# Triton-AI/Triton-Racer-Sim

Hardware: AMD Instinct MI355X
Metric: env-steps/s (whole node) at N envs x 120x160 RGB (higher is better)
Workload: dtype f32 state / f64 nearest-point / u8 image; 1 GPU; 1024 envs/GPU x 1 GPU, bicycle physics + L1 nearest point + 120x160 RGB pinhole rasteriser = BASELINE configs[2], generated_track 1185 pts, synthetic controls seed 0x5EED, auto-reset; envs_total=1024, envs_per_gpu=1024, img_h=120, img_w=160, depth=False, steps_per_launch=1, step_mode=resident worker (posted steps), prewarm_steps=8400, launcher=self

## Files before the change

triton-racer-sim_amd/csrc/trsim_plan.hpp:

```cpp
#pragma once
#include <cstddef>
#include <string>
#include <vector>

#include "trsim_tables.hpp"

#ifndef TRS_RASTER_WAVES
#define TRS_RASTER_WAVES 8
#endif

namespace trsim {

constexpr int kRasterThreads = 64 * TRS_RASTER_WAVES;
constexpr int kPhysBlock = 256;
constexpr int kCamDepth = 4;
constexpr int kSlotWords = 20;
constexpr int kLensPalBytes = 513 * 16;
constexpr int kDynTabWords = 512 + 768 + 4 + 256;

using Variant = unsigned;
constexpr Variant kVDepth = 1, kVDyn = 2, kVHills = 4, kVLens = 8, kVLight = 16, kVariants = 32;
constexpr Variant variant_bits(bool depth, bool dyn, bool hills, bool lens, bool light)
{
    return (depth ? kVDepth : 0u) | (dyn ? kVDyn : 0u) | (hills ? kVHills : 0u) | (lens ? kVLens : 0u) | (light ? kVLight : 0u);
}
constexpr bool variant_built(Variant v) { return !((v & kVDyn) && (v & kVHills)) && !((v & kVLens) && (v & (kVDyn | kVHills | kVLight))); }

inline Variant variant_clash(Variant state, Variant add)
{
    if (variant_built(state | add)) return 0;
    for (const Variant b : {kVHills, kVDyn, kVLens, kVLight})
        if ((state & b) && !variant_built(add | b)) return b;
    return 0;
}
inline const char* variant_refusal(Variant add, Variant set)
{
    struct Text { Variant add, set; const char* text; };
    static const Text kTexts[] = {
        {kVHills, kVLens, "this track has elevation and a lens camera is set: the lens camera is built for flat tracks only (trs_set_camera(NULL) first); the handle keeps its track"},
        {kVHills, kVDyn, "this track has elevation: the dynamic-brightness frame filter that was set has been removed (a frame's palette is evaluated per env inside the kernels there; "
                         "the static filter works, or use trs_preprocess on the rendered frames)"},
        {kVDyn, kVHills, "the loaded track has elevation: a frame's palette is evaluated per env inside the kernels there, and the dynamic-brightness filter behind the "
                         "rasteriser is not built for that; the static filter works, or use trs_preprocess on the rendered frames"},
        {kVDyn, kVLens, "a lens camera is set: the dynamic-brightness filter behind the rasteriser is not built for the lens camera (trs_set_camera(NULL) first); "
                        "the static filter works, or use trs_preprocess on the rendered frames"},
        {kVLens, kVHills, "the loaded track has elevation: the lens camera is built for flat tracks only (the ground plane of a hilly track tilts per env and frame)"},
        {kVLens, kVDyn, "the dynamic-brightness frame filter is set: it is not built for the lens camera (trs_set_frame_filter without dynamic brightness, or NULL, first)"},
        {kVLens, kVLight, "scene lighting is set: it is not built for the lens camera (trs_set_lighting(NULL) first)"},
        {kVLight, kVLens, "a lens camera is set: scene lighting is not built for the lens camera (trs_set_camera(NULL) first)"},
    };
    for (const Text& t : kTexts)
        if (t.add == add && t.set == set) return t.text;
    return "";
}

constexpr int kHillRowBytes = 28;
constexpr int kHillBatchMax = 4;
TRS_HD inline int hill_table_bytes(int H) { return (kHillRowBytes * H + 15) & ~15; }
TRS_HD inline int hill_batch(int H) { const int b = kRasterThreads / (H > 0 ? H : 1); return b < 1 ? 1 : (b > kHillBatchMax ? kHillBatchMax : b); }
TRS_HD inline int hill_lds_bytes(int H) { return hill_batch(H) * hill_table_bytes(H) + 48; }

constexpr int kDynBatch = 4;
TRS_HD inline int light_copies(int gpr) { return (gpr + 63 + 63) / 64; }
TRS_HD inline int light_pal_bytes(int H, int gpr) { return light_copies(gpr) * H * 16; }
TRS_HD inline int light_lds_extra(int H, int W, int slots, bool hilly, bool dyn)
{
    return slots * 32 + (hilly ? 0 : (dyn ? kDynBatch * H * 16 : light_pal_bytes(H, W / 4)));
}
TRS_HD inline int dyn_lds_bytes(int H) { return kDynBatch * H * 16 + 128 + ((kDynTabWords * 4 + 15) & ~15) + H * 16; }

TRS_HD inline int imax(int a, int b) { return (a > b) ? a : b; }
struct StepLds { int cam, prog, pitch, hill, light, dyn, total; };
TRS_HD inline int tabs_lds_bytes(int H, Variant v) { return (v & kVHills) ? hill_lds_bytes(H) : ((v & kVLens) ? kLensPalBytes : 0); }
TRS_HD inline StepLds step_lds_behind(int prog, int epw, int H, Variant v, int n_phys)
{
    const int rows = imax(n_phys, 1) + 1;
    StepLds L;
    L.prog = prog;
    L.cam = prog - rows * epw * 16;
    L.pitch = L.prog + epw * 4 + 16;
    L.hill = (L.pitch + rows * epw * 4 + 15) & ~15;
    L.light = (L.hill + tabs_lds_bytes(H, v) + 15) & ~15;
    return L;
}
TRS_HD inline StepLds step_lds_layout(int lds_step, int epw, int H, int W, Variant v, int n_phys)
{
    StepLds L = step_lds_behind(lds_step + (imax(n_phys, 1) + 1) * epw * 16, epw, H, v, n_phys);
    int end = L.pitch;
    if (v & (kVHills | kVLens | kVLight)) end = L.hill + tabs_lds_bytes(H, v);
    if (v & kVLight) end = L.light + light_lds_extra(H, W, epw, (v & kVHills) != 0, (v & kVDyn) != 0);
    L.dyn = (end + 15) & ~15;
    L.total = (v & kVDyn) ? L.dyn + dyn_lds_bytes(H) : end;
    return L;
}

TRS_HD inline size_t wlds_slot_off(int epw) { return (64 + (size_t)epw * 8 + 15) & ~(size_t)15; }
TRS_HD inline size_t wlds_bytes(int epw)
{
    return wlds_slot_off(epw) + (size_t)kCamDepth * epw * kSlotWords * 4 + (size_t)epw * 64;
}

struct WorkerLds { int ctl, dyn, hill, light, total; };
TRS_HD inline int worker_lds_light(int hill, int H, Variant v) { return (hill + tabs_lds_bytes(H, v) + 15) & ~15; }
TRS_HD inline WorkerLds worker_lds_layout(int lds_step, int epw, int H, int W, Variant v)
{
    WorkerLds L;
    L.ctl = (lds_step + 15) & ~15;
    int end = (int)(L.ctl + wlds_bytes(epw) + 16);
    L.dyn = (end + 15) & ~15;
    if (v & kVDyn) end = L.dyn + dyn_lds_bytes(H);
    L.hill = (end + 15) & ~15;
    if (v & (kVHills | kVLens)) end = L.hill + tabs_lds_bytes(H, v);
    L.light = worker_lds_light(L.hill, H, v);
    L.total = (v & kVLight) ? L.light + light_lds_extra(H, W, kCamDepth * epw, (v & kVHills) != 0, (v & kVDyn) != 0) : end;
    return L;
}

inline int steps_that_fit(int lds_step, int epw, int H, int W, Variant v)
{
    int n = 0;
    while (n < 16 && step_lds_layout(lds_step, epw, H, W, v, n + 1).total <= 160 * 1024) ++n;
    return n;
}
inline bool resident_fits(int lds_step, int epw, int H, int W, Variant v) { return worker_lds_layout(lds_step, epw, H, W, v).total <= 160 * 1024; }
enum class LdsFit { ok, no_launch, no_worker };
inline LdsFit lds_fit(int lds_step, int epw, int H, int W, Variant v, bool resident)
{
    if (steps_that_fit(lds_step, epw, H, W, v) < 1) return LdsFit::no_launch;
    return resident && !resident_fits(lds_step, epw, H, W, v) ? LdsFit::no_worker : LdsFit::ok;
}

constexpr bool variant_keeps_uniform(Variant v) { return !(v & (kVDyn | kVLens | kVLight)); }
struct UniformRows {
    bool ok[2] = {false, false};
    void invalidate() { ok[0] = ok[1] = false; }
    unsigned skip_mask(Variant v) const { return variant_keeps_uniform(v) ? (ok[0] ? 1u : 0u) | (ok[1] ? 2u : 0u) : 0u; }
    void rendered(Variant v, unsigned long long first, unsigned long long n)
    {
        for (unsigned long long k = 0; k < n && k < 2; ++k) ok[(first + k) & 1ull] = variant_keeps_uniform(v);
    }
};

TRS_HD inline bool worker_skips_uniform(unsigned mask, unsigned long long start, unsigned long long s) { return ((mask >> (s & 1ull)) & 1u) != 0 || s - start >= 2; }
TRS_HD inline int worker_step_stores(int nstep, int nuni, bool skips) { return skips ? nstep - nuni : nstep; }
TRS_HD inline int worker_wait_count(unsigned mask, unsigned long long start, unsigned long long owed, unsigned long long s, int nstep, int nuni, int uni_now)
{
    int n = uni_now;
    for (unsigned long long q = owed + 1; q < s; ++q) n += worker_step_stores(nstep, nuni, worker_skips_uniform(mask, start, q));
    return n;
}
TRS_HD inline int worker_lag(int nstep, int nuni, bool skipping) { return (2 * worker_step_stores(nstep, nuni, skipping) + (skipping ? 0 : nuni) <= 63) ? 3 : 2; }

struct TrackLayout {
    struct Phys { int off_py, off_pz, off_tan, tan_in_lds, off_gstart, off_gpts, blob_bytes, off_scratch, pts_bytes, lds_p; } p;
    struct Raster { int map_pitch_b, off_rowtab, off_pal, off_depth, off_sky, blob_bytes, lds_r; } r;
    int lds_off_phys, lds_step;
};
int track_layout(const TrackTables& T, int H, bool render, int envs_per_wg, TrackLayout& L, std::string& err);
void pack_track_images(const TrackTables& T, int H, const TrackLayout& L, std::vector<unsigned char>& phys, std::vector<unsigned char>& raster);

}
```

triton-racer-sim_amd/csrc/trsim_resident.hip:

```cpp
#include <hip/hip_runtime.h>

#include <algorithm>
#include <array>
#include <atomic>
#include <chrono>
#include <cstdint>
#include <cstdlib>
#include <cstddef>
#include <cstring>
#include <mutex>
#include <string>
#include <utility>

#include "../../include/trsim.h"
#include "../../include/trsim_spec.h"
#include "trsim_device.hpp"
#include "trsim_env.hpp"
#include "trsim_internal.hpp"

#define TRS_EXPORT extern "C" __attribute__((visibility("default")))

namespace trsim {

constexpr int kSlots = 8;
// ... 220 lines not shown
        seen = ok ? (want | 0x100u) : expected;
    }
    seen = (unsigned)__builtin_amdgcn_readfirstlane((int)seen);
    won = (seen & 0x100u) != 0u;
    return seen & 0xffu;
}

__device__ __forceinline__ void leave_not_coresident(const WParams& wp, const WLds& l, int lane, bool won)
{
    if (won) {
        if (lane == 0) sys_store64(&wp.mb->consumed, wp.start);
        drain_vmem();
        if (lane == 0) sys_store64(&wp.mb->exited, kExitNotCoresident);
    }
    dispatcher_publish_exit(wp, l, wp.start, lane);
}

__device__ __forceinline__ int dispatcher_checkin(const WParams& wp, const WLds& l, int lane)
{
    const u64 t0 = (u64)wall_clock64();
    bool cancel = sys_load64(&wp.mb->close) == kCloseCancel, won = false;
    for (unsigned spins = 0; !cancel; ++spins) {
        if (decision_load(wp) == kNoGo) { leave_not_coresident(wp, l, lane, false); return 0; }
        if (__hip_atomic_load(&wp.dc->checkin[0], __ATOMIC_RELAXED, __HIP_MEMORY_SCOPE_AGENT) >= (unsigned)wp.n_blocks) {
            if (decision_close(wp, kGo, lane, won) != kGo) { leave_not_coresident(wp, l, lane, false); return 0; }
            if (lane == 0) sys_store64(&wp.mb->started, 1ull);
            return 1;
        }
        if (agent_load64(&wp.dc->word) & kAbortBit) {
            if (lane == 0) __hip_atomic_fetch_or(l.word, kAbortBit, __ATOMIC_RELAXED, __HIP_MEMORY_SCOPE_WORKGROUP);
            return 0;
        }
        if ((u64)wall_clock64() - t0 > wp.checkin_ticks) break;
        if ((spins & 63u) == 63u) cancel = sys_load64(&wp.mb->close) == kCloseCancel;
        __builtin_amdgcn_s_sleep(4);
    }
    const unsigned d = decision_close(wp, kNoGo, lane, won);
    if (d == kGo) { if (lane == 0) sys_store64(&wp.mb->started, 1ull); return 1; }
    leave_not_coresident(wp, l, lane, won);
    return 0;
}

__device__ __forceinline__ int leader_wait_decision(const WParams& wp, const WLds& l, int lane)
{
    const u64 t0 = (u64)wall_clock64();
    for (;;) {
        unsigned d = decision_load(wp);
        if (d == 0u && (u64)wall_clock64() - t0 > 2ull * wp.checkin_ticks) {
            bool won = false;
            d = decision_close(wp, kNoGo, lane, won);
            if (d == kNoGo) { leave_not_coresident(wp, l, lane, won); return 0; }
        }
        if (d == kGo) return 1;
        if (d == kNoGo) { leave_not_coresident(wp, l, lane, false); return 0; }
        if (agent_load64(&wp.dc->word) & kAbortBit) {
            if (lane == 0) __hip_atomic_fetch_or(l.word, kAbortBit, __ATOMIC_RELAXED, __HIP_MEMORY_SCOPE_WORKGROUP);
            return 0;
        }
        __builtin_amdgcn_s_sleep(8);
    }
}

__device__ __forceinline__ void dispatcher_run(const WParams& wp, const WLds& l, int lane)
{
    if (!dispatcher_checkin(wp, l, lane)) return;
    Leader L{wp.start, (u64)wall_clock64(), (u64)wall_clock64()};
    for (;;) {
        if ((lds_load64(l.word) | agent_load64(&wp.dc->word)) & kAbortBit) {
            if (lane == 0) __hip_atomic_fetch_or(l.word, kAbortBit, __ATOMIC_RELAXED, __HIP_MEMORY_SCOPE_WORKGROUP);
            return;
        }
        const u64 now = (u64)wall_clock64();
        bool close_req = false;
        const int fresh = dispatcher_take(wp, l, L, lane, close_req);
        const bool busy = (u64)lds_load64(l.fwd) < L.known;
        if (fresh || busy) L.t_last = now;
        const bool leave = (!fresh && (close_req || now - L.t_last > wp.idle_ticks)) || now - L.t_start > wp.life_ticks;
        if (!leave) { if (!fresh) __builtin_amdgcn_s_sleep(4); continue; }
        if (lane == 0) sys_store64(&wp.mb->exited, kExitNormal);
        drain_vmem();
        (void)dispatcher_take(wp, l, L, lane, close_req);
        if (lane == 0) sys_store64(&wp.mb->consumed, L.known);
        dispatcher_publish_exit(wp, l, L.known, lane);
        return;
    }
}

__device__ __forceinline__ void raster_arrive(const WLds& l, u64 s, int lane)
{
    if (lane == 0) __hip_atomic_fetch_add(&l.arrive[s & (kSlots - 1)], 1, __ATOMIC_RELAXED, __HIP_MEMORY_SCOPE_WORKGROUP);
}

__device__ __forceinline__ void forward_arrivals(const WParams& wp, const WLds& l, u64& fwd, int lane, int want = kRasterThreads / 64)
{
    const int slot = (int)(fwd & (kSlots - 1));
    if (lds_load32(&l.arrive[slot]) != want) return;
    if (lane == 0) {
        lds_store32(&l.arrive[slot], 0);
        const int shard = (int)(blockIdx.x & 7u), nshards = min(8, wp.n_blocks);
        const unsigned members = (unsigned)((wp.n_blocks - shard + 7) / 8);
        const unsigned uses = (unsigned)((fwd - wp.start) / (u64)kSlots) + 1u;
        unsigned* a = &wp.dc->arrive[slot][shard][0];
        if (__hip_atomic_fetch_add(a, 1u, __ATOMIC_RELAXED, __HIP_MEMORY_SCOPE_AGENT) == members * uses - 1u) {
            unsigned* t = &wp.dc->top[slot][0];
            if (__hip_atomic_fetch_add(t, 1u, __ATOMIC_RELAXED, __HIP_MEMORY_SCOPE_AGENT) == (unsigned)nshards * uses - 1u)
                sys_store64(&wp.mb->done[slot], fwd + 1);
        }
    }
    fwd += 1;
    if (lane == 0) lds_store64(l.fwd, fwd);
}

struct Duties { bool leader, forwarder; u64 fwd; int want = kRasterThreads / 64; };

__device__ __forceinline__ int wait_posted(const WParams& wp, const WLds& l, Duties& D, u64 s, int lane)
{
    u64 t0 = 0;
    for (unsigned spins = 0;; ++spins) {
        if (D.forwarder) forward_arrivals(wp, l, D.fwd, lane, D.want);
        const u64 w = lds_load64(l.word);
        if (w & kAbortBit) return 0;
        if ((w & kCountMask) > s) return 1;
        if (w & kExitBit) return 0;
        if (D.leader) {
            const u64 g = agent_load64(&wp.dc->word);
            if (g != w) { if (lane == 0) lds_store64(l.word, g); drain_lds(); continue; }
        }
        __builtin_amdgcn_s_sleep(4);
        if ((spins & 255u) == 255u) {
            const u64 now = (u64)wall_clock64();
            if (t0 == 0) t0 = now;
            else if (now - t0 > wp.safety_ticks) { worker_abort(wp, l, 1u); return 0; }
        }
    }
}

__device__ __forceinline__ int wait_lds_ge(const WParams& wp, const WLds& l, Duties* D, const int* ctr, int want, unsigned code, int lane)
{
    u64 t0 = 0;
    for (unsigned spins = 0;; ++spins) {
        if (lds_load32(ctr) >= want) return 1;
        if (D && D->forwarder) forward_arrivals(wp, l, D->fwd, lane, D->want);
        __builtin_amdgcn_s_sleep(1);
        if ((spins & 1023u) == 1023u) {
            if (lds_load64(l.word) & kAbortBit) return 0;
            const u64 now = (u64)wall_clock64();
            if (t0 == 0) t0 = now;
            else if (now - t0 > wp.safety_ticks) { worker_abort(wp, l, code); return 0; }
        }
    }
}

template <bool DEPTH, bool DYN, bool HILLS = false, bool LENS = false, bool LIGHT = false>
__global__ __launch_bounds__(kBlock) void trs_worker_kernel(const WParams wp)
{
    const int tid = threadIdx.x, lane = tid & 63, wave = tid >> 6;
    const bool raster_team = tid < kRasterThreads;
    const RParams& p = wp.ra;
    const PParams& P = wp.ph;
    const int epw = p.envs_per_wg;
    const WLds l = wlds_of(smem + wp.lds_off_ctl, epw);
    const int e_begin = blockIdx.x * epw;
    const int n_loc = min(e_begin + epw, p.n_envs) - e_begin;
    const int pw = wave - kRasterThreads / 64;
    if ((unsigned)(uintptr_t)smem != 0u) {
        if (tid == 0) {
            atomicAdd(&p.stats[2], 1ull);
            sys_store64(p.fault, 1ull);
            sys_store64(&wp.mb->error, (9ull << 32) | (u64)blockIdx.x);
            __hip_atomic_fetch_or(&wp.dc->word, kAbortBit, __ATOMIC_RELAXED, __HIP_MEMORY_SCOPE_AGENT);
            if (blockIdx.x == 0) { sys_store64(&wp.mb->consumed, wp.start); sys_store64(&wp.mb->exited, 1ull); }
        }
        return;
    }
    if (raster_team) stage_lds_dma(p.blob, p.blob_bytes, 0u, wave, kRasterThreads / 64, lane);
    else stage_lds_dma(P.blob, P.blob_bytes, (unsigned)wp.lds_off_phys, pw, kPhysWaves, lane);
    if (LENS && raster_team) lens_stage_palette(p, (unsigned)wp.lds_off_hill, wave, lane);
    if (tid == 0) { lds_store64(l.word, wp.start); lds_store64(l.fwd, wp.start); }
    if (tid < kSlots) l.arrive[tid] = 0;
    for (int j = tid; j < 2 * epw; j += kBlock) l.pprog[j] = 0;
    int* const hbar = reinterpret_cast<int*>(smem + wp.lds_off_hill + hill_batch(p.H) * hill_table_bytes(p.H));
    if (HILLS && tid == 0) *hbar = 0;
    const int lds_off_light = worker_lds_light(wp.lds_off_hill, p.H, variant_bits(DEPTH, DYN, HILLS, LENS, LIGHT));
    float* const lring = reinterpret_cast<float*>(smem + lds_off_light);
    const unsigned lds_off_lpal = (unsigned)lds_off_light + (unsigned)(kCamDepth * epw * 32);
    const float* const light_g = LIGHT ? reinterpret_cast<const trsim::HillBlock*>(p.blob + trsim::hill_block_offset(p.blob_bytes))->light : nullptr;
    const int lfilt = LIGHT ? reinterpret_cast<const trsim::HillBlock*>(p.blob + trsim::hill_block_offset(p.blob_bytes))->filt : 0;
    if constexpr (DYN) {
        if (tid < 32) reinterpret_cast<int*>(smem + wp.fp.lds_off + kDynBatch * p.H * 16)[tid] = 0;
        dyn_stage_tables(smem, wp.fp, p.H, tid, kBlock, reinterpret_cast<const uint32_t*>(p.blob + p.off_pal));
    }
    if (!raster_team)
        for (int j = pw; j < n_loc; j += kPhysWaves) {
            EnvRegs st;
            env_load(P, e_begin + j, st);
            const float lr = coherent_load(&P.last_return[e_begin + j]);
            if (lane == 0) {
                float* q = l.lst + (size_t)j * 16;
                q[0] = st.x; q[1] = st.y; q[2] = st.z; q[3] = st.yaw; q[4] = st.v; q[5] = st.sf; q[6] = st.epr;
                q[7] = __int_as_float(st.seg); q[8] = __int_as_float(st.epl); q[9] = __int_as_float(st.done); q[10] = __int_as_float(st.pend);
                q[11] = lr;
            }
        }
    asm volatile("s_waitcnt vmcnt(0) lgkmcnt(0)" ::: "memory");
    __syncthreads();
    if (tid == 0) worker_checkin(wp);

    if (!raster_team) {
        const int first = blockIdx.x == 0 ? 1 : 0, nphys = kPhysWaves - first;
        if (pw < first) { dispatcher_run(wp, l, lane); return; }
        Duties D{blockIdx.x != 0 && pw == 0, pw == kPhysWaves - 1, wp.start};
        if (D.leader && !leader_wait_decision(wp, l, lane)) return;
        const unsigned char* const lphys = smem + wp.lds_off_phys;
        u64 s = wp.start;
        for (;; ++s) {
            const int r = (int)(s - wp.start);
            if (!wait_posted(wp, l, D, s, lane)) break;
            const u64* en = reinterpret_cast<const u64*>(&wp.dc->ring[s & (kSlots - 1)]);
            const u64 ev = lane < 6 ? agent_load64(en + lane) : 0ull;
            const float* const c_st = reinterpret_cast<const float*>(lane_u64(ev, 1));
            const float* const c_th = reinterpret_cast<const float*>(lane_u64(ev, 2));
            const float* const c_br = reinterpret_cast<const float*>(lane_u64(ev, 3));
            const uint8_t* const c_rs = reinterpret_cast<const uint8_t*>(lane_u64(ev, 4));
            const int synth = (int)(unsigned)lane_u64(ev, 5);
            for (int j = pw - first; j < n_loc; j += nphys) {
                const int e = e_begin + j;
                if (r >= kCamDepth && !wait_lds_ge(wp, l, &D, &l.rread[j], (r - kCamDepth + 1) * (kRasterThreads / 64), 2u, lane)) return;
                float steer = 0.f, thr = 0.f, brk = 0.f;
                uint8_t rin = 0;
                if (!synth) {
                    steer = sys_load_val(&c_st[e]); thr = sys_load_val(&c_th[e]);
                    if (c_br) brk = sys_load_val(&c_br[e]);
                    if (c_rs) rin = sys_load_val(&c_rs[e]);
                }
                float* const q = l.lst + (size_t)j * 16;
                EnvRegs st;
                st.x = q[0]; st.y = q[1]; st.z = q[2]; st.yaw = q[3]; st.v = q[4]; st.sf = q[5]; st.epr = q[6];
                st.seg = __float_as_int(q[7]); st.epl = __float_as_int(q[8]); st.done = __float_as_int(q[9]); st.pend = __float_as_int(q[10]);
                st.speed = 0.f; st.cte = 0.f;
                float lr = q[11];
                const float epr_before = st.epr;
                StepOut o;
                if (n_loc <= TRS_PHYS_PRIO_MAX_ENVS) __builtin_amdgcn_s_setprio(3);
                env_advance<true, false>(P, lphys, e, st, (uint32_t)s, synth, steer, thr, brk, rin, lane, o,
                                         HILLS ? reinterpret_cast<const trsim::HillBlock*>(p.blob + trsim::hill_block_offset(p.blob_bytes)) : nullptr);
                if (n_loc <= TRS_PHYS_PRIO_MAX_ENVS) __builtin_amdgcn_s_setprio(0);
                if (o.do_reset) lr = epr_before;
                if constexpr (LIGHT) {
                    const float lv = lane < 8 ? sys_load_val(&light_g[(size_t)e * 8 + lane]) : 0.f;
                    if (lane < 8) lring[((size_t)(r & (kCamDepth - 1)) * epw + j) * 8 + lane] = lv;
                }
                if (lane == 0) {
                    q[0] = st.x; q[1] = st.y; q[2] = st.z; q[3] = st.yaw; q[4] = st.v; q[5] = st.sf; q[6] = st.epr;
                    q[7] = __int_as_float(st.seg); q[8] = __int_as_float(st.epl); q[9] = __int_as_float(st.done); q[10] = __int_as_float(st.pend);
                    q[11] = lr;
                    float* const sl = l.slot + ((size_t)(r & (kCamDepth - 1)) * epw + j) * kSlotWords;
                    *reinterpret_cast<float4*>(sl) = o.cam;
                    sl[4] = st.x; sl[5] = st.y; sl[6] = st.z; sl[7] = st.yaw; sl[8] = st.v; sl[9] = st.speed; sl[10] = st.cte;
                    sl[11] = __int_as_float(st.seg); sl[12] = st.epr; sl[13] = __int_as_float(st.epl); sl[14] = st.sf; sl[15] = lr;
                    sl[16] = __int_as_float(st.done);
                    if constexpr (HILLS) sl[17] = o.pitch;
                    if (o.is_done) atomicAdd(&P.stats[0], 1ull);
                    if (o.do_reset) atomicAdd(&P.stats[1], 1ull);
                    drain_lds();
                    lds_store32(&l.pprog[j], r + 1);
                }
            }
        }
        if (D.forwarder) {
            u64 t0 = 0;
            for (unsigned spins = 0; D.fwd < s; ++spins) {
                forward_arrivals(wp, l, D.fwd, lane);
                if (lds_load64(l.word) & kAbortBit) break;
                __builtin_amdgcn_s_sleep(2);
                if ((spins & 1023u) == 1023u) {
                    const u64 now = (u64)wall_clock64();
                    if (t0 == 0) t0 = now;
                    else if (now - t0 > wp.safety_ticks) { worker_abort(wp, l, 4u); break; }
                }
            }
        }
        return;
    }

    const RasterThread rth = raster_thread(p, smem, tid);
    trsim::LensBlock lb{};
    LensCacheWorker<DEPTH> lcache;
    if constexpr (LENS) {
        lb = *reinterpret_cast<const trsim::LensBlock*>(p.blob + trsim::lens_block_offset(p.blob_bytes));
        lens_cache_load(p, rth, lb, lcache);
    }
    int nu = 0, ng = 0;
    for (int v = rth.vstart; v < p.uni_rows; v += p.rows_per_pass) ++nu;
    for (int v = rth.vground; v < p.H; v += p.rows_per_pass) ++ng;
#pragma unroll
    for (int off = 32; off >= 1; off >>= 1) { nu = max(nu, __shfl_xor(nu, off, 64)); ng = max(ng, __shfl_xor(ng, off, 64)); }
    nu *= DEPTH ? 2 : 1; ng *= DEPTH ? 2 : 1;
    int own = 0;
    for (int j = wave; j < n_loc; j += kRasterThreads / 64) ++own;
    const int nuni = nu * n_loc, nstep = (nu + ng) * n_loc + 2 * own;
    constexpr bool kSkipUniform = !DYN && !HILLS && !LIGHT && !LENS;
    const int lag = worker_lag(nstep, nuni, kSkipUniform);
    unsigned char* optr = nullptr;
    {
        unsigned char* const tab[14] = {(unsigned char*)P.x, (unsigned char*)P.y, (unsigned char*)P.z, (unsigned char*)P.yaw, (unsigned char*)P.v,
                                        (unsigned char*)P.speed, (unsigned char*)P.cte, (unsigned char*)P.seg_idx, (unsigned char*)P.ep_return,
                                        (unsigned char*)P.ep_len, (unsigned char*)P.steer_filt, (unsigned char*)P.last_return,
                                        (unsigned char*)P.done, (unsigned char*)P.pending};
#pragma unroll
        for (int k = 0; k < 14; ++k) optr = lane == k ? tab[k] : optr;
    }
    Duties none{false, false, 0};
    u64 owed = wp.start;
    const bool probe = (kDiag & 4) && blockIdx.x == 7 && wave == 0;
    auto now_clk = [&]() -> u64 { u64 t; asm volatile("s_memtime %0\n\ts_waitcnt lgkmcnt(0)" : "=s"(t) :: "memory"); return t; };
    u64 t_post = 0, t_pose = 0, t_vm = 0, t_all = 0, t_mark = probe ? now_clk() : 0;
    for (u64 s = wp.start;; ++s) {
        const int r = (int)(s - wp.start);
        if (owed < s && (lds_load64(l.word) & kCountMask) <= s) {
            drain_vmem();
            for (; owed < s; ++owed) raster_arrive(l, owed, lane);
        }
        const u64 tp0 = probe ? now_clk() : 0;
        if (!wait_posted(wp, l, none, s, lane)) {
            drain_vmem();
            for (; owed < s; ++owed) raster_arrive(l, owed, lane);
            if (probe && lane == 0) {
                t_all = now_clk() - t_mark;
                atomicAdd(&p.stats[40], t_post); atomicAdd(&p.stats[41], t_pose); atomicAdd(&p.stats[42], t_vm); atomicAdd(&p.stats[43], t_all);
                atomicAdd(&p.stats[44], (u64)r);
            }
            return;
        }
        if (probe) t_post += now_clk() - tp0;
        uint8_t* const img = (s & 1ull) ? wp.img1 : wp.img0;
        float* const dep = (s & 1ull) ? wp.dep1 : wp.dep0;
        const u64 ahead = (lds_load64(l.word) & kCountMask) - 1 - s;
        const u64 keep = ahead + 1 < (u64)lag ? ahead + 1 : (u64)lag;
        if constexpr (DYN) {
            while (s - owed >= keep) {
                wait_vmcnt_le((int)(s - owed - 1) * nstep);
                raster_arrive(l, owed++, lane);
            }
            const int nbatch = (n_loc + kDynBatch - 1) / kDynBatch;
            for (int b0 = 0; b0 < n_loc; b0 += kDynBatch) {
                float4 cams[kDynBatch];
                unsigned tel = 0; int mine_j = -1;
#pragma unroll
                for (int bi = 0; bi < kDynBatch; ++bi) {
                    const int j = b0 + bi;
                    cams[bi] = make_float4(0.f, 0.f, 0.f, 1.f);
                    if (j < n_loc) {
                        if (!wait_lds_ge(wp, l, nullptr, &l.pprog[j], r + 1, 3u, lane)) return;
                        const float* const sl = l.slot + ((size_t)(r & (kCamDepth - 1)) * epw + j) * kSlotWords;
                        cams[bi] = *reinterpret_cast<const float4*>(sl);
                        if ((j % (kRasterThreads / 64)) == wave) { mine_j = j; tel = __float_as_uint(sl[4 + min(lane, 12)]); }
                        asm volatile("s_waitcnt lgkmcnt(0)" :: "v"(cams[bi].x), "v"(cams[bi].y), "v"(cams[bi].z), "v"(cams[bi].w), "v"(tel) : "memory");
                        if (!LIGHT && lane == 0) __hip_atomic_fetch_add(&l.rread[j], 1, __ATOMIC_RELAXED, __HIP_MEMORY_SCOPE_WORKGROUP);
                    }
                }
                u64 t0_bar = 0;
                auto bail = [&](bool first) -> bool {
                    if (lds_load64(l.word) & kAbortBit) return true;
                    const u64 now = (u64)wall_clock64();
                    if (first) { t0_bar = now; return false; }
                    if (now - t0_bar > wp.safety_ticks) { worker_abort(wp, l, 5u); return true; }
                    return false;
                };
                if (!raster_dyn_batch<DEPTH, LIGHT>(p, wp.fp, rth, smem, cams, min(kDynBatch, n_loc - b0), img, dep, e_begin + b0, r * nbatch + b0 / kDynBatch, tid, lane, bail,
                                                   LIGHT ? lring + ((size_t)(r & (kCamDepth - 1)) * epw + b0) * 8 : nullptr, lds_off_lpal)) return;
                if (LIGHT && lane == 0)
                    for (int bi = 0; bi < kDynBatch && b0 + bi < n_loc; ++bi) __hip_atomic_fetch_add(&l.rread[b0 + bi], 1, __ATOMIC_RELAXED, __HIP_MEMORY_SCOPE_WORKGROUP);
                if (mine_j >= 0 && !(kDiag & 2)) {
                    const size_t e = (size_t)(e_begin + mine_j);
                    if (lane < 12) __hip_atomic_store((__attribute__((address_space(1))) unsigned*)(uintptr_t)optr + e, tel, __ATOMIC_RELAXED, __HIP_MEMORY_SCOPE_SYSTEM);
                    else if (lane < 14) __hip_atomic_store((__attribute__((address_space(1))) unsigned char*)(uintptr_t)optr + e, (unsigned char)(lane == 12 ? tel : 0u), __ATOMIC_RELAXED, __HIP_MEMORY_SCOPE_SYSTEM);
                }
            }
            continue;
        }
        if constexpr (HILLS) {
            while (s - owed >= keep) {
                wait_vmcnt_le((int)(s - owed - 1) * nstep);
                raster_arrive(l, owed++, lane);
            }
            const int HB = hill_batch(p.H);
            const int nbatch = (n_loc + HB - 1) / HB;
            for (int b0 = 0; b0 < n_loc; b0 += HB) {
                const int nb = min(HB, n_loc - b0);
                float4 cams[kHillBatchMax]; float Pv[kHillBatchMax];
                unsigned tel = 0; int mine_j = -1;
#pragma unroll
                for (int bi = 0; bi < kHillBatchMax; ++bi) {
                    cams[bi] = make_float4(0.f, 0.f, 0.f, 1.f); Pv[bi] = 0.f;
                    const int j = b0 + bi;
                    if (bi < nb) {
                        if (!wait_lds_ge(wp, l, nullptr, &l.pprog[j], r + 1, 3u, lane)) return;
                        const float* const sl = l.slot + ((size_t)(r & (kCamDepth - 1)) * epw + j) * kSlotWords;
                        cams[bi] = *reinterpret_cast<const float4*>(sl);
                        Pv[bi] = sl[17];
                        if ((j % (kRasterThreads / 64)) == wave) { mine_j = j; tel = __float_as_uint(sl[4 + min(lane, 12)]); }
                        asm volatile("s_waitcnt lgkmcnt(0)" :: "v"(cams[bi].x), "v"(cams[bi].y), "v"(cams[bi].z), "v"(cams[bi].w), "v"(tel), "v"(Pv[bi]) : "memory");
                        if (!LIGHT && lane == 0) __hip_atomic_fetch_add(&l.rread[j], 1, __ATOMIC_RELAXED, __HIP_MEMORY_SCOPE_WORKGROUP);
                    }
                }
                u64 t0_bar = 0;
                auto bail = [&](bool first) -> bool {
                    if (lds_load64(l.word) & kAbortBit) return true;
                    const u64 now = (u64)wall_clock64();
                    if (first) { t0_bar = now; return false; }
                    if (now - t0_bar > wp.safety_ticks) { worker_abort(wp, l, 5u); return true; }
                    return false;
                };
                const int done_before = (r * nbatch + b0 / HB) * 2 * (kRasterThreads / 64);
                if (!hill_batch_build(p, smem, (unsigned)wp.lds_off_hill, Pv, nb, hbar, done_before, tid, lane, bail,
                                      LIGHT ? lring + ((size_t)(r & (kCamDepth - 1)) * epw + b0) * 8 : nullptr)) return;
                if (LIGHT && lane == 0)
                    for (int bi = 0; bi < nb; ++bi) __hip_atomic_fetch_add(&l.rread[b0 + bi], 1, __ATOMIC_RELAXED, __HIP_MEMORY_SCOPE_WORKGROUP);
#pragma unroll
                for (int bi = 0; bi < kHillBatchMax; ++bi)
// ... 160 lines not shown
        const float* const c_th = reinterpret_cast<const float*>(lane_u64(ev, 2));
        const float* const c_br = reinterpret_cast<const float*>(lane_u64(ev, 3));
        const uint8_t* const c_rs = reinterpret_cast<const uint8_t*>(lane_u64(ev, 4));
        Ctl in{0.f, 0.f, 0.f, 0, (int)(unsigned)lane_u64(ev, 5)};
        asm volatile("" :: "s"(c_st), "s"(c_th), "s"(in.synth) : "memory");
        if (!in.synth) {
            in.steer = sys_load_val(&c_st[e]); in.thr = sys_load_val(&c_th[e]);
            if (c_br) in.brk = sys_load_val(&c_br[e]);
            if (c_rs) in.rin = sys_load_val(&c_rs[e]);
        }
        return in;
    };
    bool have_ctl = false, have_ent = false;
    Ctl nxt{};
    u64 ent_next = 0ull;
    u64 clean_below = wp.start;
    for (u64 s = wp.start;; ++s) {
        if (owed < s && (lds_load64(l.word) & kCountMask) <= s) {
            drain_vmem();
            for (; owed < s; ++owed) raster_arrive(l, owed, lane);
            clean_below = s;
        }
        Ctl in;
        if (have_ctl) {
            in = nxt;
        } else {
            if (!wait_posted(wp, l, none, s, lane)) {
                drain_vmem();
                for (; owed < s; ++owed) raster_arrive(l, owed, lane);
                return;
            }
            in = ctl_load(entry_load(s));
            drain_vmem();
            clean_below = s;
        }
        const u64 count = lds_load64(l.word) & kCountMask;
        have_ctl = count > s + 1;
        if (have_ctl) {
            const bool was_prefetched = have_ent;
            nxt = ctl_load(was_prefetched ? ent_next : entry_load(s + 1));
            const u64 c = was_prefetched ? s - 1 : s;
            clean_below = c > clean_below ? c : clean_below;
        }
        have_ent = have_ctl && count > s + 2;
        if (have_ent) ent_next = entry_load(s + 2);
        for (; owed < clean_below; ++owed) raster_arrive(l, owed, lane);
        const float epr_before = st.epr;
        StepOut o;
        env_advance<true, false, true>(P, smem, e, st, (uint32_t)s, in.synth, in.steer, in.thr, in.brk, in.rin, lane, o);
        if (o.do_reset) lr = epr_before;
        if (lane == 0) {
            if (o.is_done) atomicAdd(&P.stats[0], 1ull);
            if (o.do_reset) atomicAdd(&P.stats[1], 1ull);
        }
        unsigned tel = 0;
        {
            const unsigned vals[13] = {__float_as_uint(st.x), __float_as_uint(st.y), __float_as_uint(st.z), __float_as_uint(st.yaw), __float_as_uint(st.v),
                                       __float_as_uint(st.speed), __float_as_uint(st.cte), (unsigned)st.seg, __float_as_uint(st.epr), (unsigned)st.epl,
                                       __float_as_uint(st.sf), __float_as_uint(lr), (unsigned)st.done};
#pragma unroll
            for (int k = 0; k < 13; ++k) tel = lane == k ? vals[k] : tel;
        }
        if (lane < 12) __hip_atomic_store((__attribute__((address_space(1))) unsigned*)(uintptr_t)optr + e, tel, __ATOMIC_RELAXED, __HIP_MEMORY_SCOPE_SYSTEM);
        else if (lane < 14) __hip_atomic_store((__attribute__((address_space(1))) unsigned char*)(uintptr_t)optr + e, (unsigned char)(lane == 12 ? tel : 0u), __ATOMIC_RELAXED, __HIP_MEMORY_SCOPE_SYSTEM);
    }
}

__global__ void trs_worker_init_kernel(DevCtl* dc, u64 start)
{
    unsigned* w = reinterpret_cast<unsigned*>(dc);
    for (int i = threadIdx.x; i < (int)(sizeof(DevCtl) / 4); i += blockDim.x) w[i] = 0u;
    __syncthreads();
    if (threadIdx.x == 0) agent_store64(&dc->word, start);
}


#define RCHK(call)                                                                                \
    do {                                                                                          \
        hipError_t _e = (call);                                                                   \
        if (_e != hipSuccess) return trs_internal_fail(TRS_ERR_DEVICE, std::string(#call) + ": " + hipGetErrorString(_e)); \
    } while (0)

inline uint64_t host_load(const uint64_t* p) { return __atomic_load_n(p, __ATOMIC_ACQUIRE); }
inline void host_store(uint64_t* p, uint64_t v) { __atomic_store_n(p, v, __ATOMIC_RELEASE); }

int worker_fits(trs_env* e)
{
    Resident* R = e->res;
    if (!e->cfg.render) {
        R->lds_off_ctl = (e->lds_p + 15) & ~15;
        R->lds_bytes = (int)(R->lds_off_ctl + wlds_bytes(kPwEnvs) + 16);
        if (R->lds_bytes > 160 * 1024) return trs_internal_fail(TRS_ERR_LIMIT, "track image too large for the resident physics worker");
        if (R->pw_capacity_lds != R->lds_bytes) {
            int per_cu = 0;
            RCHK(hipOccupancyMaxActiveBlocksPerMultiprocessor(&per_cu, reinterpret_cast<const void*>(trs_physics_worker_kernel), kPwBlock, (size_t)R->lds_bytes));
            R->pw_capacity_envs = (long long)per_cu * (long long)std::max(e->cu_count, 1) * kPwEnvs;
            R->pw_capacity_lds = R->lds_bytes;
        }
        const long long capacity = R->pw_capacity_envs / kPwEnvs;
        const long long grid = ((long long)e->n + kPwEnvs - 1) / kPwEnvs;
        if (capacity > 0 && grid > capacity)
            return trs_internal_fail(TRS_ERR_LIMIT, "resident mode: " + std::to_string(e->n) + " physics-only envs need " + std::to_string(grid) +
                                                        " co-resident workgroups, this GPU holds " + std::to_string(capacity) + " (" + std::to_string(capacity * kPwEnvs) +
                                                        " envs): use TRS_STEP_LAUNCH with several steps per launch for shards of this size");
        return TRS_OK;
    }
    const WorkerLds L = worker_lds_layout(e->lds_step, e->pp.envs_per_wg, e->H, e->W, variant_of(e));
    R->lds_off_ctl = L.ctl; R->lds_off_dyn = L.dyn; R->lds_off_hill = L.hill; R->lds_bytes = L.total;
    if (R->lds_bytes > 160 * 1024)
        return trs_internal_fail(TRS_ERR_LIMIT, e->hilly ? "the resident worker's LDS state and the per-env row tables of a track with elevation do not fit beside this track's tables: use TRS_STEP_LAUNCH"
                                                : e->lens_on ? "the resident worker's LDS state and the lens camera's palette do not fit beside this track's tables: use TRS_STEP_LAUNCH"
                                                : e->light_on ? "the resident worker's LDS state and the lit palettes of scene lighting do not fit beside this track's tables: use TRS_STEP_LAUNCH"
                                                            : "too many envs per workgroup for the resident worker's LDS state");
    return TRS_OK;
}

int evict(trs_env* other);

int worker_launch(trs_env* e, uint64_t start)
{
    Resident* R = e->res;
    Mailbox* mb = R->mb.get();
    { int rc = worker_fits(e); if (rc) return rc; }
    const WorkerKernel kernel = e->cfg.render ? kWorkerKernels[variant_of(e)] : nullptr;
    if (e->cfg.render && !kernel)
        return trs_internal_fail(TRS_ERR_STATE, "internal error: no resident worker is built for this combination of camera, track, frame filter and lighting");
    {
        DeviceSlot& D = slot_of(e);
        trs_env* const other = D.owner;
        if (other && other != e && other->res && other->res->running) (void)evict(other);
        D.owner = e;
    }
    host_store(&mb->exited, 0); host_store(&mb->consumed, start); host_store(&mb->error, 0);
    host_store(&mb->close, 0); host_store(&mb->started, 0);
    WParams wp{};
    wp.ph = e->pp; wp.ph.synth = 0; wp.ph.write_cam = 0; wp.ph.n_steps = 0; wp.ph.step_off = 0; wp.ph.ctl_stride = 0;
    wp.ra = e->rp;
    wp.img0 = e->img[0].get(); wp.img1 = e->img[1].get(); wp.dep0 = e->depth[0].get(); wp.dep1 = e->depth[1].get();
    wp.uni_mask = e->cfg.render ? e->uniform_ok.skip_mask(variant_of(e)) : 0u;
    R->gen_start = start; R->gen_variant = e->cfg.render ? variant_of(e) : 0u;
    wp.mb = mb; wp.dc = R->dc.get();
    wp.start = start;
    wp.idle_ticks = (unsigned long long)R->idle_us * 100ull;
    wp.life_ticks = (unsigned long long)R->life_us * 100ull;
    wp.safety_ticks = 200000000ull;
    wp.checkin_ticks = 200000ull;
    wp.lds_off_phys = e->lds_off_phys; wp.lds_off_ctl = R->lds_off_ctl; wp.lds_off_hill = R->lds_off_hill;
    const int grid = e->cfg.render ? (e->n + e->pp.envs_per_wg - 1) / e->pp.envs_per_wg : (e->n + kPwEnvs - 1) / kPwEnvs;
    wp.n_blocks = grid;
    if (!(R->dc_ready && R->dc_ready_for == start)) hipLaunchKernelGGL(trs_worker_init_kernel, dim3(1), dim3(256), 0, e->sP, R->dc.get(), (u64)start);
    R->dc_ready = false;
    if (e->cfg.render) {
        wp.fp = fparams_of(e, R->lds_off_dyn);
        hipLaunchKernelGGL(kernel, dim3(grid), dim3(kBlock), R->lds_bytes, e->sP, wp);
    } else {
        hipLaunchKernelGGL(trs_physics_worker_kernel, dim3(grid), dim3(kPwBlock), R->lds_bytes, e->sP, wp);
    }
    RCHK(hipGetLastError());
    R->running = true;
    R->t_launch = std::chrono::steady_clock::now();
    return TRS_OK;
}

void worker_rendered(trs_env* e, uint64_t consumed)
{
    Resident* R = e->res;
    if (e->cfg.render && consumed > R->gen_start) e->uniform_ok.rendered(R->gen_variant, R->gen_start, consumed - R->gen_start);
    R->gen_start = std::max(R->gen_start, consumed);
}

int worker_error(trs_env* e)
{
    const uint64_t err = host_load(&e->res->mb->error);
    if (!err) return TRS_OK;
    e->res->broken = true;
    e->uniform_ok.invalidate();
    static const char* const what[] = {"", "waiting for a post", "camera ring back-pressure", "waiting for the physics team", "forwarding the last arrivals",
                                       "team barrier of the dynamic-brightness batch", "", "abort injected by trs_resident_debug_abort (test hook)", "",
                                       "dynamic LDS segment not at offset 0"};
    const unsigned code = (unsigned)(err >> 32);
    return trs_internal_fail(TRS_ERR_DEVICE, std::string("resident worker gave up (") + (code < 10 ? what[code] : "?") + ") in workgroup " +
                                                 std::to_string((unsigned)err));
}

int fall_back_to_launches(trs_env* e, uint64_t consumed, const char* why)
{
    Resident* R = e->res;
    const uint64_t posted = host_load(&R->mb->posted);
    R->enabled = false;
    R->fell_back = true;
    R->t_fallback = std::chrono::steady_clock::now();
    if (consumed > R->seen_done) R->seen_done = consumed;
    for (uint64_t s = consumed; s < posted; ++s) {
        const WEntry& en = R->mb->ring[s & (kSlots - 1)];
        if (en.seq != s + 1 || en.seq_lo != s + 1)
            return trs_internal_fail(TRS_ERR_DEVICE, "resident worker: the post of step " + std::to_string(s) + " is no longer in the ring");
        int rc = trs_internal_replay_launch(e, en.steer, en.thr, en.brk, en.reset, (int)en.synth, s);
        if (rc) return rc;
    }
    R->launched = true;
    R->base = R->seen_done = e->step_count;
    for (int k = 0; k < kSlots; ++k) { host_store(&R->mb->ring[k].seq, 0); host_store(&R->mb->ring[k].seq_lo, 0); host_store(&R->mb->done[k], 0); }
    trs_internal_note(std::string("resident worker: ") + why + " - another process's worker holds CUs of this GPU; the handle has gone back to TRS_STEP_LAUNCH "
                      "(resident mode is tried again by itself after " + std::to_string(R->retry_ms) + " ms; trs_get_step_mode tells)");
    return kFellBack;
}

int handle_exit(trs_env* e, bool relaunch = true)
{
    Resident* R = e->res;
    RCHK(hipStreamSynchronize(e->sP));
    R->running = false;
    int rc = worker_error(e);
    if (rc) return rc;
    const uint64_t consumed = host_load(&R->mb->consumed), posted = host_load(&R->mb->posted);
    worker_rendered(e, consumed);
    if (host_load(&R->mb->exited) == kExitNotCoresident)
        return fall_back_to_launches(e, consumed, "the launch did not get every CU within 2 ms");
    if (consumed > R->seen_done) R->seen_done = consumed;
    if (host_load(&R->mb->started)) R->retry_ms = kRetryMs0;
    if (consumed < posted && relaunch) return worker_launch(e, consumed);
    if (consumed == posted) {
        hipLaunchKernelGGL(trs_worker_init_kernel, dim3(1), dim3(256), 0, e->sP, R->dc.get(), (u64)consumed);
        if (hipGetLastError() == hipSuccess) { R->dc_ready = true; R->dc_ready_for = consumed; }
    }
    return TRS_OK;
}

int evict(trs_env* other)
{
    Resident* R = other->res;
    int rc = TRS_OK;
    if (R->running) {
        host_store(&R->mb->close, kCloseLeave);
        rc = handle_exit(other, false);
    }
    return rc < 0 ? rc : TRS_OK;
}

int give_up_on_launch(trs_env* e)
{
    Resident* R = e->res;
    host_store(&R->mb->close, kCloseCancel);
    RCHK(hipStreamSynchronize(e->sP));
    R->running = false;
    int rc = worker_error(e);
    if (rc) return rc;
    worker_rendered(e, host_load(&R->mb->consumed));
    return fall_back_to_launches(e, host_load(&R->mb->consumed), "the launch had not started after 250 ms");
}

int wait_done(trs_env* e, uint64_t s)
{
    Resident* R = e->res;
    if (s < R->seen_done) return TRS_OK;
    Mailbox* mb = R->mb.get();
    const auto t0 = std::chrono::steady_clock::now();
    auto fell_back = [&]() -> int {
        RCHK(hipStreamSynchronize(e->sP));
        R->launched = false;
        R->base = R->seen_done = e->step_count;
        return TRS_OK;
    };
    for (unsigned spins = 0;; ++spins) {
        if (host_load(&mb->done[s & (kSlots - 1)]) >= s + 1) { R->seen_done = s + 1; return TRS_OK; }
        if ((spins & 63u) == 63u) {
            if (R->running && host_load(&mb->exited)) {
                int rc = handle_exit(e);
                if (rc == kFellBack) return fell_back();
                if (rc) return rc;
                if (s < R->seen_done) return TRS_OK;
            } else if (!R->running) {
                if (host_load(&mb->posted) > R->seen_done) { int rc = worker_launch(e, R->seen_done); if (rc) return rc; }
            } else if ((spins & 4095u) == 4095u && !host_load(&mb->started) &&
                       std::chrono::steady_clock::now() - R->t_launch > std::chrono::milliseconds(250)) {
                int rc = give_up_on_launch(e);
                if (rc == kFellBack) return fell_back();
                if (rc) return rc;
            }
            if (host_load(&mb->error)) { (void)handle_exit(e); return worker_error(e); }
            if (std::chrono::steady_clock::now() - t0 > std::chrono::seconds(10))
                return trs_internal_fail(TRS_ERR_DEVICE, "resident worker: step " + std::to_string(s) + " did not complete within 10 s");
        }
        __builtin_ia32_pause();
    }
}

int ensure_resident(trs_env* e)
{
    Resident* R = e->res;
    if (R->mb.get()) return TRS_OK;
    RCHK(R->mb.alloc(sizeof(Mailbox), hipHostMallocMapped | hipHostMallocCoherent));
    std::memset(R->mb.get(), 0, sizeof(Mailbox));
    RCHK(R->dc.alloc(sizeof(DevCtl)));
    {
        int least = 0, greatest = 0;
        RCHK(hipDeviceGetStreamPriorityRange(&least, &greatest));
        RCHK(hipStreamCreateWithPriority(&R->sC, hipStreamNonBlocking, greatest));
    }
    R->hctl_slot = ((size_t)e->n * 13 + 63) & ~(size_t)63;
    RCHK(R->hctl.alloc(R->hctl_slot * kSlots, hipHostMallocMapped | hipHostMallocCoherent));
    return TRS_OK;
}

}

namespace trsim {
// ... 232 lines not shown
```

Before: 125.1 million env-steps/s.

## Batch control loads per wave and add optional service wave with run-ahead prefetch

Control inputs for all envs a physics wave owns are now loaded once per step in parallel across lanes and broadcast with readlane, instead of serial per-env system loads. An optional service wave (compile-time, off by default) can take over dispatch/forwarding so physics waves prefetch the next step's ring entry and controls ahead of time. Timing probes gated by a diagnostic flag are also added. This adds code complexity and assumes at most 64 envs per wave.

```diff
diff --git a/triton-racer-sim_amd/csrc/trsim_plan.hpp b/triton-racer-sim_amd/csrc/trsim_plan.hpp
--- a/triton-racer-sim_amd/csrc/trsim_plan.hpp
+++ b/triton-racer-sim_amd/csrc/trsim_plan.hpp
@@ -116,6 +116,40 @@
     return L;
 }
 
+#ifndef TRS_PHYS_WAVES
+#define TRS_PHYS_WAVES 4
+#endif
+#ifndef TRS_WORKER_SERVICE_WAVES
+#define TRS_WORKER_SERVICE_WAVES 0
+#endif
+#ifndef TRS_WORKER_AHEAD
+#define TRS_WORKER_AHEAD 1
+#endif
+constexpr int kStepWaves = TRS_RASTER_WAVES + TRS_PHYS_WAVES;
+constexpr int kWorkerServiceWaves = TRS_WORKER_SERVICE_WAVES;
+static_assert(kWorkerServiceWaves == 0 || kWorkerServiceWaves == 1, "one service wave, or none");
+constexpr bool worker_has_service_wave(Variant v) { return kWorkerServiceWaves > 0 && !(v & (kVDyn | kVHills | kVLens)); }
+constexpr int worker_waves(Variant v) { return kStepWaves + (worker_has_service_wave(v) ? kWorkerServiceWaves : 0); }
+constexpr int worker_block(Variant v) { return 64 * worker_waves(v); }
+constexpr bool worker_runs_ahead(Variant v) { return TRS_WORKER_AHEAD != 0 && worker_has_service_wave(v); }
+enum class WorkerRole { raster, physics, dispatcher, service, none };
+constexpr WorkerRole worker_role(Variant v, int wg, int wave)
+{
+    if (wave < 0 || wave >= worker_waves(v)) return WorkerRole::none;
+    if (wave < TRS_RASTER_WAVES) return WorkerRole::raster;
+    if (wave >= kStepWaves) return wg == 0 ? WorkerRole::dispatcher : WorkerRole::service;
+    return !worker_has_service_wave(v) && wg == 0 && wave == TRS_RASTER_WAVES ? WorkerRole::dispatcher : WorkerRole::physics;
+}
+constexpr int worker_first_env_wave(Variant v, int wg) { return !worker_has_service_wave(v) && wg == 0 ? 1 : 0; }
+constexpr int worker_env_waves(Variant v, int wg) { return TRS_PHYS_WAVES - worker_first_env_wave(v, wg); }
+constexpr int worker_envs_of_wave(Variant v, int wg, int pw, int n_loc)
+{
+    const int first = worker_first_env_wave(v, wg), waves = worker_env_waves(v, wg), k = pw - first;
+    return k < 0 || k >= n_loc ? 0 : (n_loc - k + waves - 1) / waves;
+}
+constexpr bool worker_phys_leads(Variant v, int wg, int pw) { return !worker_has_service_wave(v) && wg != 0 && pw == 0; }
+constexpr bool worker_phys_forwards(Variant v, int wg, int pw) { return (!worker_has_service_wave(v) || wg == 0) && pw == TRS_PHYS_WAVES - 1; }
+
 inline int steps_that_fit(int lds_step, int epw, int H, int W, Variant v)
 {
     int n = 0;
diff --git a/triton-racer-sim_amd/csrc/trsim_resident.hip b/triton-racer-sim_amd/csrc/trsim_resident.hip
--- a/triton-racer-sim_amd/csrc/trsim_resident.hip
+++ b/triton-racer-sim_amd/csrc/trsim_resident.hip
@@ -396,8 +396,11 @@
 }
 
 template <bool DEPTH, bool DYN, bool HILLS = false, bool LENS = false, bool LIGHT = false>
-__global__ __launch_bounds__(kBlock) void trs_worker_kernel(const WParams wp)
-{
+__global__ __launch_bounds__(worker_block(variant_bits(DEPTH, DYN, HILLS, LENS, LIGHT))) void trs_worker_kernel(const WParams wp)
+{
+    constexpr Variant kV = variant_bits(DEPTH, DYN, HILLS, LENS, LIGHT);
+    constexpr int kWBlock = worker_block(kV);
+    constexpr bool kService = worker_has_service_wave(kV), kAhead = worker_runs_ahead(kV);
     const int tid = threadIdx.x, lane = tid & 63, wave = tid >> 6;
     const bool raster_team = tid < kRasterThreads;
     const RParams& p = wp.ra;
@@ -418,11 +421,11 @@
         return;
     }
     if (raster_team) stage_lds_dma(p.blob, p.blob_bytes, 0u, wave, kRasterThreads / 64, lane);
-    else stage_lds_dma(P.blob, P.blob_bytes, (unsigned)wp.lds_off_phys, pw, kPhysWaves, lane);
+    else stage_lds_dma(P.blob, P.blob_bytes, (unsigned)wp.lds_off_phys, pw, kWBlock / 64 - kRasterThreads / 64, lane);
     if (LENS && raster_team) lens_stage_palette(p, (unsigned)wp.lds_off_hill, wave, lane);
     if (tid == 0) { lds_store64(l.word, wp.start); lds_store64(l.fwd, wp.start); }
     if (tid < kSlots) l.arrive[tid] = 0;
-    for (int j = tid; j < 2 * epw; j += kBlock) l.pprog[j] = 0;
+    for (int j = tid; j < 2 * epw; j += kWBlock) l.pprog[j] = 0;
     int* const hbar = reinterpret_cast<int*>(smem + wp.lds_off_hill + hill_batch(p.H) * hill_table_bytes(p.H));
     if (HILLS && tid == 0) *hbar = 0;
     const int lds_off_light = worker_lds_light(wp.lds_off_hill, p.H, variant_bits(DEPTH, DYN, HILLS, LENS, LIGHT));
@@ -432,9 +435,9 @@
     const int lfilt = LIGHT ? reinterpret_cast<const trsim::HillBlock*>(p.blob + trsim::hill_block_offset(p.blob_bytes))->filt : 0;
     if constexpr (DYN) {
         if (tid < 32) reinterpret_cast<int*>(smem + wp.fp.lds_off + kDynBatch * p.H * 16)[tid] = 0;
-        dyn_stage_tables(smem, wp.fp, p.H, tid, kBlock, reinterpret_cast<const uint32_t*>(p.blob + p.off_pal));
-    }
-    if (!raster_team)
+        dyn_stage_tables(smem, wp.fp, p.H, tid, kWBlock, reinterpret_cast<const uint32_t*>(p.blob + p.off_pal));
+    }
+    if (!raster_team && pw < kPhysWaves)
         for (int j = pw; j < n_loc; j += kPhysWaves) {
             EnvRegs st;
             env_load(P, e_begin + j, st);
@@ -451,32 +454,95 @@
     if (tid == 0) worker_checkin(wp);
 
     if (!raster_team) {
-        const int first = blockIdx.x == 0 ? 1 : 0, nphys = kPhysWaves - first;
+        if (kService && pw >= kPhysWaves) {
+            if (blockIdx.x == 0) { dispatcher_run(wp, l, lane); return; }
+            Duties D{true, true, wp.start};
+            if (!leader_wait_decision(wp, l, lane)) return;
+            u64 s = wp.start;
+            while (wait_posted(wp, l, D, s, lane)) ++s;
+            const u64 w = lds_load64(l.word);
+            if (w & kAbortBit) return;
+            const u64 last = w & kCountMask;
+            u64 t0 = 0;
+            for (unsigned spins = 0; D.fwd < last; ++spins) {
+                forward_arrivals(wp, l, D.fwd, lane);
+                if (lds_load64(l.word) & kAbortBit) break;
+                __builtin_amdgcn_s_sleep(2);
+                if ((spins & 1023u) == 1023u) {
+                    const u64 now = (u64)wall_clock64();
+                    if (t0 == 0) t0 = now;
+                    else if (now - t0 > wp.safety_ticks) { worker_abort(wp, l, 4u); break; }
+                }
+            }
+            return;
+        }
+        const int first = worker_first_env_wave(kV, (int)blockIdx.x), nphys = worker_env_waves(kV, (int)blockIdx.x);
         if (pw < first) { dispatcher_run(wp, l, lane); return; }
-        Duties D{blockIdx.x != 0 && pw == 0, pw == kPhysWaves - 1, wp.start};
+        Duties D{worker_phys_leads(kV, (int)blockIdx.x, pw), worker_phys_forwards(kV, (int)blockIdx.x, pw), wp.start};
         if (D.leader && !leader_wait_decision(wp, l, lane)) return;
         const unsigned char* const lphys = smem + wp.lds_off_phys;
-        u64 s = wp.start;
-        for (;; ++s) {
-            const int r = (int)(s - wp.start);
-            if (!wait_posted(wp, l, D, s, lane)) break;
-            const u64* en = reinterpret_cast<const u64*>(&wp.dc->ring[s & (kSlots - 1)]);
-            const u64 ev = lane < 6 ? agent_load64(en + lane) : 0ull;
+        const bool pprobe = (kDiag & 8) && (blockIdx.x == 7 || blockIdx.x == 0) && pw == first;
+        auto pclk = [&]() -> u64 { u64 t; asm volatile("s_memtime %0\n\ts_waitcnt lgkmcnt(0)" : "=s"(t) :: "memory"); return t; };
+        u64 pt[6] = {0, 0, 0, 0, 0, 0}, pt_mark = pprobe ? pclk() : 0;
+        struct Ctl { float steer, thr, brk; unsigned rin; int synth; };
+        const int j_lane = pw - first + lane * nphys;
+        auto entry_load = [&](u64 sq) -> u64 {
+            const u64* en = reinterpret_cast<const u64*>(&wp.dc->ring[sq & (kSlots - 1)]);
+            return lane < 6 ? agent_load64(en + lane) : 0ull;
+        };
+        auto ctl_load = [&](u64 ev) -> Ctl {
             const float* const c_st = reinterpret_cast<const float*>(lane_u64(ev, 1));
             const float* const c_th = reinterpret_cast<const float*>(lane_u64(ev, 2));
             const float* const c_br = reinterpret_cast<const float*>(lane_u64(ev, 3));
             const uint8_t* const c_rs = reinterpret_cast<const uint8_t*>(lane_u64(ev, 4));
-            const int synth = (int)(unsigned)lane_u64(ev, 5);
-            for (int j = pw - first; j < n_loc; j += nphys) {
+            Ctl in{0.f, 0.f, 0.f, 0u, (int)(unsigned)lane_u64(ev, 5)};
+            if (!in.synth && j_lane < n_loc) {
+                const int e = e_begin + j_lane;
+                in.steer = sys_load_val(&c_st[e]); in.thr = sys_load_val(&c_th[e]);
+                if (c_br) in.brk = sys_load_val(&c_br[e]);
+                if (c_rs) in.rin = sys_load_val(&c_rs[e]);
+            }
+            return in;
+        };
+        bool have_ctl = false, have_ent = false;
+        Ctl nxt{};
+        u64 ent_next = 0ull;
+        u64 s = wp.start;
+        for (;; ++s) {
+            const int r = (int)(s - wp.start);
+            Ctl in;
+            if (kAhead && have_ctl) {
+                in = nxt;
+                if (D.forwarder) forward_arrivals(wp, l, D.fwd, lane, D.want);
+            } else {
+                u64 c0 = pprobe ? pclk() : 0;
+                if (!wait_posted(wp, l, D, s, lane)) break;
+                if (pprobe) { const u64 c1 = pclk(); pt[0] += c1 - c0; c0 = c1; }
+                const u64 ev = entry_load(s);
+                if (pprobe) { asm volatile("s_waitcnt vmcnt(0)" :: "v"(ev) : "memory"); const u64 c1 = pclk(); pt[1] += c1 - c0; c0 = c1; }
+                in = ctl_load(ev);
+                if (pprobe) { asm volatile("s_waitcnt vmcnt(0)" :: "v"(in.steer), "v"(in.thr), "v"(in.brk), "v"(in.rin) : "memory"); pt[2] += pclk() - c0; }
+            }
+            if constexpr (kAhead) {
+                const u64 w = lds_load64(l.word);
+                if (w & kAbortBit) break;
+                const u64 count = w & kCountMask;
+                have_ctl = count > s + 1;
+                if (have_ctl) nxt = ctl_load(have_ent ? ent_next : entry_load(s + 1));
+                have_ent = have_ctl && count > s + 2;
+                if (have_ent) ent_next = entry_load(s + 2);
+            }
+            int k = 0;
+            for (int j = pw - first; j < n_loc; j += nphys, ++k) {
                 const int e = e_begin + j;
+                const u64 b0 = pprobe ? pclk() : 0;
                 if (r >= kCamDepth && !wait_lds_ge(wp, l, &D, &l.rread[j], (r - kCamDepth + 1) * (kRasterThreads / 64), 2u, lane)) return;
-                float steer = 0.f, thr = 0.f, brk = 0.f;
-                uint8_t rin = 0;
-                if (!synth) {
-                    steer = sys_load_val(&c_st[e]); thr = sys_load_val(&c_th[e]);
-                    if (c_br) brk = sys_load_val(&c_br[e]);
-                    if (c_rs) rin = sys_load_val(&c_rs[e]);
-                }
+                const u64 b1 = pprobe ? pclk() : 0;
+                const float steer = __int_as_float(__builtin_amdgcn_readlane(__float_as_int(in.steer), k));
+                const float thr = __int_as_float(__builtin_amdgcn_readlane(__float_as_int(in.thr), k));
+                const float brk = __int_as_float(__builtin_amdgcn_readlane(__float_as_int(in.brk), k));
+                const uint8_t rin = (uint8_t)__builtin_amdgcn_readlane((int)in.rin, k);
+                const int synth = in.synth;
                 float* const q = l.lst + (size_t)j * 16;
                 EnvRegs st;
                 st.x = q[0]; st.y = q[1]; st.z = q[2]; st.yaw = q[3]; st.v = q[4]; st.sf = q[5]; st.epr = q[6];
@@ -490,6 +556,8 @@
                                          HILLS ? reinterpret_cast<const trsim::HillBlock*>(p.blob + trsim::hill_block_offset(p.blob_bytes)) : nullptr);
                 if (n_loc <= TRS_PHYS_PRIO_MAX_ENVS) __builtin_amdgcn_s_setprio(0);
                 if (o.do_reset) lr = epr_before;
+                u64 b2 = 0;
+                if (pprobe) { asm volatile("" :: "v"(st.x), "v"(st.yaw), "v"(o.cam.x) : "memory"); b2 = pclk(); }
                 if constexpr (LIGHT) {
                     const float lv = lane < 8 ? sys_load_val(&light_g[(size_t)e * 8 + lane]) : 0.f;
                     if (lane < 8) lring[((size_t)(r & (kCamDepth - 1)) * epw + j) * 8 + lane] = lv;
@@ -509,7 +577,13 @@
                     drain_lds();
                     lds_store32(&l.pprog[j], r + 1);
                 }
-            }
+                if (pprobe) { pt[3] += b1 - b0; pt[4] += b2 - b1; pt[5] += pclk() - b2; }
+            }
+        }
+        if (pprobe && lane == 0) {
+            unsigned long long* const out = &P.stats[blockIdx.x == 7 ? 8 : 16];
+            for (int i = 0; i < 6; ++i) atomicAdd(&out[i], pt[i]);
+            atomicAdd(&out[6], pclk() - pt_mark); atomicAdd(&out[7], s - wp.start);
         }
         if (D.forwarder) {
             u64 t0 = 0;
@@ -976,7 +1050,7 @@
     R->dc_ready = false;
     if (e->cfg.render) {
         wp.fp = fparams_of(e, R->lds_off_dyn);
-        hipLaunchKernelGGL(kernel, dim3(grid), dim3(kBlock), R->lds_bytes, e->sP, wp);
+        hipLaunchKernelGGL(kernel, dim3(grid), dim3(worker_block(variant_of(e))), R->lds_bytes, e->sP, wp);
     } else {
         hipLaunchKernelGGL(trs_physics_worker_kernel, dim3(grid), dim3(kPwBlock), R->lds_bytes, e->sP, wp);
     }
```

After: 122.7 million env-steps/s. 1.9% lower.
